# czbiohub-sf/yogo

Measured on AMD Instinct MI355X. Metric: training images/sec (772x1032 gray), higher is better.
Workload: dtype bf16; 1 GPU; BASELINE configs[2]: full train step (fwd+loss+bwd+clamp+AdamW), base_model, 772x1032x1 uint8, 7 classes; per_gpu_batch=128, global_batch=128, parallelism=dp1

## Files before the change

### include/yogo_hip.h

```cpp
#ifndef YOGO_HIP_H
#define YOGO_HIP_H

#include <stddef.h>

#ifdef __cplusplus
extern "C" {
#endif

typedef void* yogo_stream_t;

const char* yogo_hip_last_error(void);
int yogo_hip_abi_version(void);
int yogo_hip_launch_log(int enable);
int yogo_hip_launch_log_read(char* buf, size_t cap, size_t* needed);


int yogo_conv_packed_bytes(int Cin, int Cout, int ksize, int stride, int mode, size_t* bytes);
int yogo_conv_pack_f32(const float* w_oihw, float* packed, int Cin, int Cout, int ksize, int stride, int mode,
                       yogo_stream_t stream);
int yogo_conv2d_fwd_stats_shape(int B, int Cin, int Cout, int IH, int IW, int ksize, int stride, int* rows, int* mpad);
int yogo_conv2d_fwd_f32(const float* in, const float* packed, const float* bias, float* out, float* out_pre,
                        const float* chan_scale, float* stats_part, int B, int Cin, int Cout, int IH, int IW, int ksize,
                        int stride, int act, yogo_stream_t stream);
int yogo_conv2d_dgrad_f32(const float* dy, const float* packed_dgrad, float* dx, const float* act_ref, int ref_act,
// ... 54 lines not shown
                                     yogo_stream_t stream);
int yogo_head1x1_decode_fwd_bf16(const void* x, const void* packed, const float* bias, float* out, const float* cxs, const float* cys,
                                 int B, int Cin, int P, int Sy, int Sx, float anchor_w, float anchor_h, float width_multiplier,
                                 float height_multiplier, int inference, yogo_stream_t stream);

int yogo_match_workspace_bytes(int B, int Sy, int Sx, int cap, size_t* bytes);
int yogo_match_preds_labels_batched(const float* rows, const int* counts, const float* labels, int* meta, int* pair_label,
                                    int* pair_pred, int* un_label, int* un_pred, float* lab_out, void* workspace, int B, int P, int Sy,
                                    int Sx, int cap, yogo_stream_t stream);
int yogo_match_gather(const float* rows, const float* lab_out, const int* meta, const int* pair_label, const int* pair_pred,
                      const int* un_label, const int* un_pred, float* preds, float* labels, float* missed, float* extra, int B, int P,
                      int cap, long long K, long long Km, long long Ke, yogo_stream_t stream);
int yogo_metrics_state_layout(int C, int T, int nbins, long long* offsets);
int yogo_metrics_accumulate(const float* rows, const float* lab_out, const int* meta, const int* pair_label, const int* pair_pred,
                            const int* un_label, const int* un_pred, const double* roc_thresholds, int T, const double* cal_edges,
                            int nbins, long long* acc, double* bin_conf, double* partial, float* map_rows, long long map_cap, int B,
                            int P, int cap, yogo_stream_t stream);

int yogo_bf16_channel_blocks(int C);
int yogo_conv_bf16_packed_bytes(int Cin, int Cout, int ksize, int mode, size_t* bytes);
int yogo_conv_bf16_pack(const float* w_oihw, const float* scale, void* packed, int Cin, int Cout, int ksize, int mode,
                        yogo_stream_t stream);
int yogo_conv2d_fwd_bf16_stats_shape(int B, int Cin, int Cout, int IH, int IW, int ksize, int stride, int* rows, int* mpad);
int yogo_conv2d_fwd_bf16(const void* in, const void* packed, const float* bias, void* out, float* out_f32,
                         const float* chan_scale, float* stats_part, int B, int Cin, int Cout, int IH, int IW, int ksize,
                         int stride, int act, yogo_stream_t stream);
int yogo_conv2d_fwd_bf16_pre(const void* in, const void* packed, const float* bias, void* out, void* out_pre,
                             const float* chan_scale, int B, int Cin, int Cout, int IH, int IW, int ksize, int stride, int act,
                             yogo_stream_t stream);
int yogo_conv_bf16_pack_blocks(int Cin, int Cout, int ksize, int mode, int* blocks);
int yogo_conv_bf16_pack_multi(const void* table, int n, int total_blocks, yogo_stream_t stream);
int yogo_bf16_signs_bytes(int B, int C, int H, int W, size_t* bytes);
int yogo_conv2d_fwd_bf16_signs(const void* in, const void* packed, const float* bias, void* out, void* signs,
                               const float* chan_scale, int B, int Cin, int Cout, int IH, int IW, int ksize, int stride, int act,
                               yogo_stream_t stream);
int yogo_conv2d_dgrad_bf16_signs(const void* dy, const void* packed_dgrad, void* dx, const void* signs,
                                 const float* chan_scale, int B, int Cin, int Cout, int IH, int IW, int ksize, int stride,
                                 yogo_stream_t stream);
int yogo_conv2d_dgrad_bf16(const void* dy, const void* packed_dgrad, void* dx, const void* act_ref, int ref_act,
                           const float* chan_scale, int B, int Cin, int Cout, int IH, int IW, int ksize, int stride,
                           yogo_stream_t stream);
int yogo_conv2d_wgrad_bf16in(const void* x, const void* g, float* dw, float* db, void* workspace, int B, int Cin, int Cout,
                             int IH, int IW, int ksize, int stride, float clip, yogo_stream_t stream);
int yogo_conv2d_wgrad_bf16_workspace_bytes(int B, int Cin, int Cout, int IH, int IW, int ksize, int stride, size_t* bytes);
int yogo_conv2d_wgrad_bf16(const void* x, const void* g, float* dw, float* db, void* workspace, int B, int Cin, int Cout,
                           int IH, int IW, int ksize, int stride, float clip, yogo_stream_t stream);
// ... 102 lines not shown
```

### yogo_amd/csrc/conv_bf16.hip

```cpp
#include "common.h"
#include "conv_bf16_ws.h"
#include "conv_bf16_ws16.h"
#include "conv_bf16_ws3.h"
#include <type_traits>
#include <utility>
#include <cstdlib>
#include <vector>

typedef float f32x16 __attribute__((ext_vector_type(16)));
typedef __bf16 bf16x8 __attribute__((ext_vector_type(8)));
typedef __bf16 bf16x4 __attribute__((ext_vector_type(4)));
typedef unsigned int u32x4 __attribute__((ext_vector_type(4)));
typedef unsigned int u32x2 __attribute__((ext_vector_type(2)));
typedef int i32x16 __attribute__((ext_vector_type(16)));

#define BF_MAX_TAPS 9
#define BF_LDS_BUDGET (80 * 1024)
#define BF_LDS_MAX (160 * 1024)

struct ConvBf16Params {
  const u32x4* in;
  const u32x4* wp;
  const float* bias;
  u32x2* out;
// ... 1211 lines not shown
      if constexpr (REF != 1) {
        if (!general) {
          bf_launch_one<MW, NW, NWV, S2D, PF, F32, REF, true, true>(grid, lds_bytes, stream, p, plan_txt);
          return;
        }
      }
#else
      (void)general;
#endif
      bf_launch_one<MW, NW, NWV, S2D, PF, F32, REF, true>(grid, lds_bytes, stream, p, plan_txt);
      return;
    }
  }
  if constexpr (NWV == 4 && S2D && !F32 && REF != 1) {
    const bool general = p.stats_part != nullptr || p.act == ACT_SILU || p.out_pre != nullptr || (REF == 2 && p.ref_act != ACT_LEAKY);
    if (!general) {
      bf_launch_one<MW, NW, NWV, S2D, PF, F32, REF, false, true>(grid, lds_bytes, stream, p, plan_txt);
      return;
    }
  }
  bf_launch_one<MW, NW, NWV, S2D, PF, F32, REF, false>(grid, lds_bytes, stream, p, plan_txt);
}

int launch_conv_bf16(const void* in, const void* packed, const float* bias, void* out, float* out_f32, void* out_pre, const void* act_ref,
                     int ref_act, void* signs, bool signs_read, const float* chan_scale, float* stats_part, int B, int K, int M, int IH, int IW, int OH,
                     int OW, int ks, int a, int s2d, int act, hipStream_t stream, int* stats_rows, int* stats_mpad) {
  const int T = ks * ks, pad = ks == 3 ? 1 : 0;
  if (in != nullptr && g_bf_ws && !s2d && a == 1 && ks == 3 && out_f32 == nullptr && out_pre == nullptr && act_ref == nullptr && !signs_read &&
      stats_part == nullptr && (act == ACT_NONE || act == ACT_LEAKY) && !(signs != nullptr && act != ACT_LEAKY) &&
      conv_bf16_ws_eligible(K, M, IH, IW, B)) {
    ConvWsParams q{};
    q.in = in; q.wp = packed; q.bias = bias; q.out = out; q.signs = reinterpret_cast<unsigned char*>(signs); q.chan_scale = chan_scale;
    q.B = B; q.Kb = bf_kb_of(K); q.IH = IH; q.IW = IW; q.act = act;
#ifdef YOGO_DIAG
    q.dbg = g_diag_dbg;
    q.stamps = (g_diag_stamps != nullptr && g_diag_stamps_bytes >= 512 * 128) ? g_diag_stamps : nullptr;
    if (q.stamps) (void)hipMemsetAsync(g_diag_stamps, 0, 512 * 128, stream);
#endif
    if (conv_bf16_ws_plan(&q)) {
      if ((g_bf_ws16 == 2 || (g_bf_ws16 == 1 && bias == nullptr)) && act == ACT_NONE && signs == nullptr && chan_scale == nullptr &&
          conv_bf16_ws16_eligible(K, M, IH, IW, B))
        return launch_conv_bf16_ws16(q, stream);
      return launch_conv_bf16_ws(q, stream);
    }
  }
  if (in != nullptr && g_bf_ws && !s2d && a == 2 && ks == 3 && out_f32 == nullptr && out_pre == nullptr && act_ref == nullptr && !signs_read &&
      stats_part == nullptr && (act == ACT_NONE || act == ACT_LEAKY) && !(signs != nullptr && act != ACT_LEAKY) && conv_bf16_ws3_eligible(K, M, IH, IW, B)) {
    ConvWs3Params q{};
    q.in = in; q.wp = packed; q.bias = bias; q.out = out; q.signs = reinterpret_cast<unsigned char*>(signs); q.chan_scale = chan_scale;
    q.B = B; q.Kb = bf_kb_of(K); q.IH = IH; q.IW = IW; q.OH = OH; q.OW = OW; q.act = act;
#ifdef YOGO_DIAG
    q.dbg = g_diag_dbg;
    q.stamps = (g_diag_stamps != nullptr && g_diag_stamps_bytes >= 512 * 128) ? g_diag_stamps : nullptr;
    if (q.stamps) (void)hipMemsetAsync(g_diag_stamps, 0, 512 * 128, stream);
#endif
    if (conv_bf16_ws3_plan(&q)) return launch_conv_bf16_ws3(q, stream);
  }
  if (in != nullptr && g_bf_head && ks == 1 && a == 1 && !s2d && out_pre == nullptr && act_ref == nullptr && stats_part == nullptr && act == ACT_NONE &&
      out_f32 != nullptr && out == nullptr && signs == nullptr && chan_scale == nullptr && conv_bf16_head_fwd_eligible(K, M, OH * OW, B))
    return launch_conv_bf16_head_fwd(in, packed, bias, out_f32, B, K, M, OH * OW, stream);
  if (in != nullptr && g_bf_staged && !s2d && ks == 3 && out_f32 == nullptr && out_pre == nullptr && act_ref == nullptr && !signs_read && stats_part == nullptr &&
      (act == ACT_NONE || act == ACT_LEAKY) && !(signs != nullptr && act != ACT_LEAKY) && conv_bf16_staged_eligible(K, M, a, IH, IW, OH, OW, B))
    return launch_conv_bf16_staged(in, packed, bias, out, signs, chan_scale, B, K, M, IH, IW, OH, OW, a, act, stream);
  if (in != nullptr && g_bf_direct && s2d && ks == 3 && out_f32 == nullptr && out_pre == nullptr && act_ref == nullptr && bias == nullptr &&
      stats_part == nullptr && act == ACT_NONE && (!signs_read || (signs != nullptr && ref_act == ACT_LEAKY)) && (signs_read || signs == nullptr) &&
      conv_bf16_s2d_direct_eligible(K, M, OH, OW, B))
    return launch_conv_bf16_s2d_direct(in, packed, out, signs_read ? signs : nullptr, chan_scale, B, K, M, IH, IW, OH, OW, stream);
  const int MW = bf_pick_mw(M);
  const bool small_n = s2d || a == 2;
  const bool wide64 = MW == 2 && !small_n && K >= 64 && OH * OW >= 4096;
  const int NW = MW == 1 ? (small_n ? 2 : 4) : (small_n ? 1 : (wide64 ? 4 : 2));
  const int NWV = (MW == 4 || wide64) ? 8 : 4;
  const int PF = NWV == 8 ? 10 : 16;
  const int Kb = bf_kb_of(K), Mpad = bf_mpad_of(M);
  const int OHt = s2d ? (OH + 1) / 2 : OH, OWt = s2d ? (OW + 1) / 2 : OW;
  BfTiling tl;
  bool planned = false;
  if (NWV == 4) {
    const int ladder[3] = {40 * 1024, 53 * 1024, BF_LDS_BUDGET};
// ... 101 lines not shown
    else if (MW == 2) BFLAUNCH(2, 1, 4, false, 16);
    else BFLAUNCH(1, 2, 4, false, 16);
  } else {
    if (MW == 4) BFLAUNCH(4, 2, 8, false, 10);
    else if (MW == 2 && wide64) BFLAUNCH(2, 4, 8, false, 10);
    else if (MW == 2) BFLAUNCH(2, 2, 4, false, 16);
    else BFLAUNCH(1, 4, 4, false, 16);
  }
#undef BFLAUNCH
#undef BFLAUNCH_
#undef BFLAUNCH__
  YOGO_CHECK_LAUNCH("conv_bf16");
  return YOGO_OK;
}

int check_bf16_conv(int B, int Cin, int Cout, int IH, int IW, int ks, int stride) {
  YOGO_CHECK_ARG((ks == 3 || ks == 1) && (stride == 1 || stride == 2) && !(ks == 1 && stride != 1) && B >= 0 && Cin > 0 &&
                     Cout > 0 && IH > 0 && IW > 0, "conv_bf16: unsupported shape");
  return YOGO_OK;
}

}

extern "C" int yogo_conv2d_fwd_bf16_stats_shape(int B, int Cin, int Cout, int IH, int IW, int ks, int stride, int* rows, int* mpad) {
  if (int e = check_bf16_conv(B, Cin, Cout, IH, IW, ks, stride)) return e;
  const int pad = ks == 3 ? 1 : 0;
  return launch_conv_bf16(nullptr, nullptr, nullptr, nullptr, nullptr, nullptr, nullptr, 0, nullptr, false, nullptr, nullptr, B, Cin, Cout, IH, IW,
                          (IH + 2 * pad - ks) / stride + 1, (IW + 2 * pad - ks) / stride + 1, ks, stride, 0, 0, nullptr, rows, mpad);
}

extern "C" int yogo_conv2d_fwd_bf16(const void* in, const void* packed, const float* bias, void* out, float* out_f32,
                                    const float* chan_scale, float* stats_part, int B, int Cin, int Cout, int IH, int IW,
                                    int ks, int stride, int act, hipStream_t stream) {
  YOGO_CHECK_ARG(in && packed && (out || out_f32), "conv2d_fwd_bf16: null pointer");
  if (int e = check_bf16_conv(B, Cin, Cout, IH, IW, ks, stride)) return e;
  const int pad = ks == 3 ? 1 : 0;
  return launch_conv_bf16(in, packed, bias, out, out_f32, nullptr, nullptr, 0, nullptr, false, chan_scale, stats_part, B, Cin, Cout, IH, IW,
                          (IH + 2 * pad - ks) / stride + 1, (IW + 2 * pad - ks) / stride + 1, ks, stride, 0, act, stream,
                          nullptr, nullptr);
}

extern "C" int yogo_conv2d_fwd_bf16_pre(const void* in, const void* packed, const float* bias, void* out, void* out_pre,
                                        const float* chan_scale, int B, int Cin, int Cout, int IH, int IW, int ks, int stride,
                                        int act, hipStream_t stream) {
  YOGO_CHECK_ARG(in && packed && out && out_pre, "conv2d_fwd_bf16_pre: null pointer");
  if (int e = check_bf16_conv(B, Cin, Cout, IH, IW, ks, stride)) return e;
// ... 65 lines not shown
```

### yogo_amd/csrc/conv_bf16_ws3.h

```cpp
#pragma once
#include "common.h"

#define W3_PT 128
#define W3_ROWS 9
#define W3_PL 48
#define W3_LW (2 * W3_PL)
#define W3_KBU (W3_ROWS * W3_LW)
#define W3_IB (2 * W3_KBU * 16)
#define W3_NI 7
#define W3_WB (9 * 4096)
#define W3_I0 (2 * W3_WB)
#define W3_EB (W3_I0 + 3 * W3_IB)
#define W3_ES (W3_EB + 512)
#define W3_LDS_BYTES (W3_ES + 1024)

struct ConvWs3Params {
  const void* in;
  const void* wp;
  const float* bias;
  void* out;
  unsigned char* signs;
  const float* chan_scale;
  int B, Kb, IH, IW, OH, OW;
  int ncb, TW, tiles_per_band, gx, ntiles;
  int PT;
  unsigned m_gx, m_tpb, m_bw, m_bwl;
  int nchunk, act;
#ifdef YOGO_DIAG
  int dbg;
  unsigned long long* stamps;
#endif
};

bool conv_bf16_ws3_eligible(int K, int M, int IH, int IW, int B);
bool conv_bf16_ws3_plan(ConvWs3Params* p);
int launch_conv_bf16_ws3(const ConvWs3Params& p, hipStream_t stream);
```

### yogo_amd/csrc/conv_bf16_ws3.hip

```cpp
#include "conv_bf16_ws3.h"
#include <mutex>
#include <type_traits>
#include <utility>

typedef unsigned int u32x4 __attribute__((ext_vector_type(4)));
typedef int i32x4 __attribute__((ext_vector_type(4)));
typedef __bf16 bf16x8 __attribute__((ext_vector_type(8)));

namespace {

__device__ __forceinline__ int w3_udivm(int n, unsigned m) { return (int)__umulhi((unsigned)n, m); }
__device__ __forceinline__ int w3_udivm1(int n, int d, unsigned m) { return d == 1 ? n : (int)__umulhi((unsigned)n, m); }
__device__ __forceinline__ int w3_lane() {
  int l;
  asm volatile("v_mbcnt_lo_u32_b32 %0, -1, 0\n\tv_mbcnt_hi_u32_b32 %0, -1, %0" : "=v"(l));
  return l;
}
__device__ __forceinline__ i32x4 w3_rsrc(const void* ptr, unsigned bytes) {
  const unsigned long long a = reinterpret_cast<unsigned long long>(ptr);
  return i32x4{(int)(unsigned)a, (int)((unsigned)(a >> 32) & 0xFFFFu), (int)bytes, 0x00020000};
}
__device__ __forceinline__ unsigned w3_u(unsigned x) { return (unsigned)__builtin_amdgcn_readfirstlane((int)x); }
__device__ __forceinline__ i32x4 w3_u4(i32x4 r) {
  return i32x4{__builtin_amdgcn_readfirstlane(r.x), __builtin_amdgcn_readfirstlane(r.y), __builtin_amdgcn_readfirstlane(r.z), __builtin_amdgcn_readfirstlane(r.w)};
}
__device__ __forceinline__ void w3_dma9(i32x4 rs, unsigned lds, int voff, unsigned soff, unsigned step) {
  unsigned so;
  rs = w3_u4(rs); lds = w3_u(lds); soff = w3_u(soff); step = w3_u(step);
#define W3_P9 "s_add_u32 m0, m0, 4096\n\ts_add_u32 %0, %0, %5\n\tbuffer_load_dwordx4 %1, %2, %0 offen lds\n\t"
  asm volatile("s_mov_b32 m0, %3\n\ts_mov_b32 %0, %4\n\ts_nop 4\n\tbuffer_load_dwordx4 %1, %2, %0 offen lds\n\t" W3_P9 W3_P9 W3_P9 W3_P9 W3_P9 W3_P9 W3_P9 W3_P9
// ... 78 lines not shown
               : "memory", W3_ACC_CLOBBER);
}
__device__ __forceinline__ void w3_k_end(const u32x4& a0, const u32x4& a1, const u32x4& b0, const u32x4& b1) {
  asm volatile(W3_MF(0, a0, b0) W3_MF(1, a0, b1) W3_MF(2, a1, b0) W3_MF(3, a1, b1) "s_nop 15\n\ts_nop 15" : : W3_OPS_IN : "memory", W3_ACC_CLOBBER);
}
template <int BIMM0, int BIMM1>
__device__ __forceinline__ void w3_k_first(u32x4& an0, u32x4& an1, u32x4& bn0, u32x4& bn1, u32x4& am0, u32x4& am1, u32x4& bm0, u32x4& bm1, unsigned pa, unsigned pb0,
                                           unsigned pb1) {
  asm volatile(W3_RD(an0, pa, z0) W3_RD(an1, pa, z512) W3_RD(bn0, pb0, bo0) W3_RD(bn1, pb1, bo0) W3_RD(am0, pa, z4096) W3_RD(am1, pa, z4608) W3_RD(bm0, pb0, bo1)
               W3_RD(bm1, pb1, bo1) "s_waitcnt lgkmcnt(4)"
               : [an0] "=&v"(an0), [an1] "=&v"(an1), [bn0] "=&v"(bn0), [bn1] "=&v"(bn1), [am0] "=&v"(am0), [am1] "=&v"(am1), [bm0] "=&v"(bm0), [bm1] "=&v"(bm1)
               : [pa] "v"(pa), [pb0] "v"(pb0), [pb1] "v"(pb1), [z0] "n"(0), [z512] "n"(512), [z4096] "n"(4096), [z4608] "n"(4608), [bo0] "n"(BIMM0), [bo1] "n"(BIMM1)
               : "memory");
}
template <int R>
__device__ __forceinline__ void w3_acc_read8(float (&r)[8]) {
  asm volatile(
      "v_accvgpr_read_b32 %0, a[%8]\n\tv_accvgpr_read_b32 %1, a[%8+1]\n\tv_accvgpr_read_b32 %2, a[%8+2]\n\tv_accvgpr_read_b32 %3, a[%8+3]\n\t"
      "v_accvgpr_read_b32 %4, a[%8+4]\n\tv_accvgpr_read_b32 %5, a[%8+5]\n\tv_accvgpr_read_b32 %6, a[%8+6]\n\tv_accvgpr_read_b32 %7, a[%8+7]"
      : "=v"(r[0]), "=v"(r[1]), "=v"(r[2]), "=v"(r[3]), "=v"(r[4]), "=v"(r[5]), "=v"(r[6]), "=v"(r[7])
      : "n"(R)
      : W3_ACC_CLOBBER);
}
__device__ constexpr int w3_bimm(int t) { return ((t / 3) * W3_LW + ((t % 3) == 1 ? 0 : W3_PL + ((t % 3) == 2 ? 1 : 0))) * 16; }

template <class F, int... I>
__device__ __forceinline__ void w3_static_for(F&& f, std::integer_sequence<int, I...>) {
  (f(std::integral_constant<int, I>{}), ...);
}

#ifdef YOGO_DIAG
#define W3_DBG(BIT) (p.dbg & (BIT))
#define W3_STAMP() __builtin_amdgcn_s_memtime()
#else
#define W3_DBG(BIT) 0
#define W3_STAMP() 0ull
#endif

}

template <int MODE>
__global__ __launch_bounds__(512) __attribute__((amdgpu_waves_per_eu(2, 2))) void conv_bf16_ws3_kernel(const ConvWs3Params p) {
  extern __shared__ __attribute__((aligned(16))) u32x4 smem4[];
  constexpr unsigned OOB = 0x80000000u;
  float* const ldsf = reinterpret_cast<float*>(smem4);
  const int tid = threadIdx.x;
  const int wave = __builtin_amdgcn_readfirstlane(tid >> 6);
// ... 10 lines not shown
  struct TileS { int b, j0, bw, p0, p1, lastband; };
  auto find_tile = [&](unsigned& k, TileS& t) __attribute__((always_inline)) -> bool {
    for (;; ++k) {
      const unsigned lin = slot + k * G;
      if (lin >= NV) return false;
      const unsigned xcd = lin & 7;
      const int widx = (int)((xcd < xr ? xcd * (xq + 1) : xr * (xq + 1) + (xcd - xr) * xq) + (lin >> 3));
      const int b = w3_udivm1(widx, p.gx, p.m_gx);
      const int bx = widx - b * p.gx;
      const int cb = w3_udivm1(bx, p.tiles_per_band, p.m_tpb);
      const int tb = bx - cb * p.tiles_per_band;
      const int j0 = cb * p.TW;
      const int bw = min(p.TW, OW - j0);
      const int NPb = OH * bw;
      const int p0 = tb * p.PT;
      if (p0 >= NPb) continue;
      t.b = b; t.j0 = j0; t.bw = bw; t.p0 = p0; t.p1 = min(p0 + p.PT, NPb); t.lastband = cb == p.ncb - 1;
      return true;
    }
  };

  unsigned k_ord = 0;
  TileS T{};
  if (!find_tile(k_ord, T)) return;
  if (tid < 128) {
    ldsf[W3_EB / 4 + tid] = p.bias != nullptr ? p.bias[tid] : 0.f;
    if (p.chan_scale == nullptr) {
      ldsf[W3_ES / 4 + tid] = 1.f;
      ldsf[W3_ES / 4 + 128 + tid] = 1.f;
    }
  }
  __syncthreads();

  if (team == 1) {
    const int lane = w3_lane();
    const int ttid = tw * 64 + lane;
    const int rowb = IW * 16, kcb = IH * IW * 16;
    const unsigned ibytes = (unsigned)p.Kb * kcb, wbytes = 9u * p.Kb * 2048u;
    const unsigned so_i = 2u * kcb;
    const unsigned wstep = (unsigned)p.Kb * 2048u;
    const i32x4 rs_w = w3_rsrc(p.wp, wbytes);
    const int lane16 = W3_DBG(4) ? (int)OOB : lane * 16;
    const bool has_scale = p.chan_scale != nullptr;
    const i32x4 rs_sc = w3_rsrc(p.chan_scale, has_scale ? (unsigned)p.B * 512u : 0u);
    auto issue_scale = [&](int b, int par) __attribute__((always_inline)) {
      if (has_scale && tw < 2) w3_dma_dword(rs_sc, (unsigned)(W3_ES + par * 512 + tw * 256), lane * 4, (unsigned)((b * 128 + tw * 64) * 4));
    };
// ... 87 lines not shown

  const int lane = w3_lane(), l31 = lane & 31, half = lane >> 5;
  const unsigned a_b0 = (unsigned)(half * 128 + mh * 64 + l31) * 16u;
  const unsigned obytes = 16u * plane16;
  unsigned pbr[2];
  int vo[2];
  auto decode_pix = [&](const TileS& t) __attribute__((always_inline)) {
    const unsigned m_bw = t.lastband ? p.m_bwl : p.m_bw;
    const int bw = t.bw;
    const int i_lo = w3_udivm1(t.p0, bw, m_bw);
#pragma unroll
    for (int n = 0; n < 2; ++n) {
      const int pp = t.p0 + (nh * 2 + n) * 32 + l31;
      const bool pv = pp < t.p1;
      const int pc = pv ? pp : (t.p1 - 1);
      const int i = w3_udivm1(pc, bw, m_bw), j = pc - i * bw;
      pbr[n] = (unsigned)(2 * (i - i_lo) * W3_LW + j + half * W3_KBU) * 16u;
      vo[n] = (pv && !W3_DBG(1)) ? (i * OW + t.j0 + j) * 16 + half * plane16 : (int)OOB;
    }
  };
  decode_pix(T);
  u32x4 A[3][2], B[3][2];
  int tpar = 0;
  auto epilogue = [&](i32x4 rs_o) __attribute__((always_inline)) {
    if constexpr ((W3_ABL & 8) != 0) return;
    [[maybe_unused]] unsigned sg[2] = {0u, 0u};
    w3_static_for([&](auto q_tag) __attribute__((always_inline)) {
      constexpr int Q = decltype(q_tag)::value, MB = Q >> 1, GP = Q & 1;
      const int cl = mh * 64 + MB * 32 + 16 * GP + 4 * half;
      const float* eb = ldsf + W3_EB / 4 + cl;
      const float4 bA = *reinterpret_cast<const float4*>(eb), bB = *reinterpret_cast<const float4*>(eb + 8);
      const float ba[8] = {bA.x, bA.y, bA.z, bA.w, bB.x, bB.y, bB.z, bB.w};
      float sa[8] = {1.f, 1.f, 1.f, 1.f, 1.f, 1.f, 1.f, 1.f}, bs[8];
      if constexpr (SCALED) {
        const float* es = ldsf + W3_ES / 4 + tpar * 128 + cl;
        const float4 sA = *reinterpret_cast<const float4*>(es), sB = *reinterpret_cast<const float4*>(es + 8);
        sa[0] = sA.x; sa[1] = sA.y; sa[2] = sA.z; sa[3] = sA.w; sa[4] = sB.x; sa[5] = sB.y; sa[6] = sB.z; sa[7] = sB.w;
      }
#pragma unroll
      for (int i = 0; i < 8; ++i) bs[i] = SCALED ? ba[i] * sa[i] : ba[i];
      const unsigned so = (unsigned)(mh * 8 + MB * 4 + GP * 2) * (unsigned)plane16;
      w3_static_for([&](auto n_tag) __attribute__((always_inline)) {
        constexpr int n = decltype(n_tag)::value;
        float v[8], r[8];
        w3_acc_read8<16 * (2 * MB + n) + 8 * GP>(r);
#pragma unroll
        for (int i = 0; i < 8; ++i) v[i] = SCALED ? fmaf(r[i], sa[i], bs[i]) : r[i] + bs[i];
        if constexpr (leaky) {
          float sv[8];
#pragma unroll
          for (int i = 0; i < 8; ++i) sv[i] = v[i] * LEAKY_SLOPE;
#pragma unroll
          for (int i = 0; i < 8; ++i) asm("v_max_f32 %0, %0, %1" : "+v"(v[i]) : "v"(sv[i]));
        }
        if constexpr (write_signs) {
          unsigned mA = 0;
#define W3_SGN(I) "v_cmp_lt_f32_e32 vcc, 0, %" #I "\n\tv_addc_co_u32_e32 %0, vcc, %0, %0, vcc\n\t"
          asm(W3_SGN(8) W3_SGN(7) W3_SGN(6) W3_SGN(5) W3_SGN(4) W3_SGN(3) W3_SGN(2) "v_cmp_lt_f32_e32 vcc, 0, %1\n\tv_addc_co_u32_e32 %0, vcc, %0, %0, vcc"
              : "+v"(mA)
              : "v"(v[0]), "v"(v[1]), "v"(v[2]), "v"(v[3]), "v"(v[4]), "v"(v[5]), "v"(v[6]), "v"(v[7])
              : "vcc");
#undef W3_SGN
          sg[n] |= mA << (8 * Q);
        }
        if (W3_DBG(2)) {
#pragma unroll
          for (int i = 0; i < 8; ++i) v[i] = r[i];
        }
        bf16x8 o;
#pragma unroll
        for (int i = 0; i < 8; ++i) o[i] = (__bf16)v[i];
        const u32x4 w = __builtin_bit_cast(u32x4, o);
        const auto r0 = __builtin_amdgcn_permlane32_swap(w.x, w.z, false, false);
        const auto r1 = __builtin_amdgcn_permlane32_swap(w.y, w.w, false, false);
        const u32x4 st = {r0[0], r1[0], r0[1], r1[1]};
        w3_store16(st, vo[n], rs_o, so);
      }, std::make_integer_sequence<int, 2>{});
    }, std::make_integer_sequence<int, 4>{});
    if constexpr (write_signs) {
      const i32x4 rs_s = w3_rsrc(p.signs + (size_t)T.b * plane * 16, (unsigned)plane * 16u);
#pragma unroll
      for (int n = 0; n < 2; ++n) {
        const int vs = vo[n] < 0 ? (int)OOB : (vo[n] >> 1) + mh * 4;
        asm volatile("s_nop 4\n\tbuffer_store_dword %0, %1, %2, 0 offen\n\ts_nop 1" ::"v"(sg[n]), "v"(vs), "s"(w3_u4(rs_s)) : "memory");
      }
    }
  };
  auto period = [&](auto first_tag, auto last_tag, unsigned pa, unsigned pan, unsigned ib, unsigned ibn) __attribute__((always_inline)) {
    constexpr bool FIRST = decltype(first_tag)::value, LASTP = decltype(last_tag)::value;
    const unsigned pb0 = pbr[0] + ib, pb1 = pbr[1] + ib;
    w3_static_for([&](auto s_tag) __attribute__((always_inline)) {
      constexpr int S = decltype(s_tag)::value;
      u32x4(&Ac)[2] = A[S % 3];
      u32x4(&Bc)[2] = B[S % 3];
      if constexpr (S < 7) {
        constexpr int S2 = S + 2;
        w3_k_rd<FIRST && S == 0, S2 * 4096, w3_bimm(S2)>(Ac[0], Ac[1], Bc[0], Bc[1], A[S2 % 3][0], A[S2 % 3][1], B[S2 % 3][0], B[S2 % 3][1], pa, pb0, pb1);
      } else if constexpr (S == 7) {
        w3_k_bar(Ac[0], Ac[1], Bc[0], Bc[1], A[2][0], A[2][1], B[2][0], B[2][1]);
      } else if constexpr (!LASTP) {
// ... 15 lines not shown
    const i32x4 rs_o = w3_rsrc(reinterpret_cast<unsigned char*>(p.out) + (size_t)T.b * obytes, obytes);
    [[maybe_unused]] const unsigned long long s0 = W3_STAMP();
    w3_k_first<w3_bimm(0), w3_bimm(1)>(A[0][0], A[0][1], B[0][0], B[0][1], A[1][0], A[1][1], B[1][0], B[1][1], (unsigned)(wpar * W3_WB) + a_b0, pbr[0] + ibo, pbr[1] + ibo);
    for (int c = 0; c < nck; ++c) {
      const unsigned pa = (unsigned)(wpar * W3_WB) + a_b0, pan = (unsigned)((wpar ^ 1) * W3_WB) + a_b0;
      const unsigned ibn = ibo == W3_I0 + 2 * W3_IB ? (unsigned)W3_I0 : ibo + W3_IB;
      if (c == 0) period(TT{}, FT{}, pa, pan, ibo, ibn);
      else if (c == nck - 1) period(FT{}, TT{}, pa, pan, ibo, ibn);
      else period(FT{}, FT{}, pa, pan, ibo, ibn);
      wpar ^= 1;
      ibo = ibn;
    }
    [[maybe_unused]] const unsigned long long s1 = W3_STAMP();
    epilogue(rs_o);
    [[maybe_unused]] const unsigned long long s2 = W3_STAMP();
    t_k += s1 - s0; t_e += s2 - s1;
    unsigned kn = k_ord + 1;
    const bool has_next = find_tile(kn, T);
    k_ord = kn;
    if (!has_next) break;
    decode_pix(T);
    tpar ^= 1;
  }
#ifdef YOGO_DIAG
  if (p.stamps && tw == 0 && lane == 0) {
    unsigned long long* d = p.stamps + (size_t)blockIdx.x * 16;
    d[0] = t_start; d[1] = __builtin_amdgcn_s_memtime(); d[2] = t_k; d[3] = t_e; d[6] = k_ord;
  }
#endif
}

bool conv_bf16_ws3_eligible(int K, int M, int IH, int IW, int B) {
  const int Kb = round_up(K, 16) / 8;
  if (M != 128 || Kb < 8 || (Kb % 4) != 0) return false;
  if (IH < 3 || IW < 3 || B <= 0) return false;
  const long long OH = (IH - 1) / 2 + 1, OW = (IW - 1) / 2 + 1;
  if ((long long)Kb * IH * IW * 16 >= (1ll << 31) || 16ll * OH * OW * 16 >= (1ll << 31)) return false;
  return true;
}

bool conv_bf16_ws3_plan(ConvWs3Params* p) {
  const int OH = p->OH, OW = p->OW;
  long long best = -1;
  int best_ncb = 0, best_pt = 0;
  for (int ncb = 1; ncb <= 64 && ncb <= OW; ++ncb) {
    const int TW = cdiv(OW, ncb);
// ... 1 lines not shown
    const int bw_min = OW - (ncb - 1) * TW;
    const int pt = OH <= 4 ? W3_PT : min(W3_PT, 3 * bw_min + 1);
    const long long tiles = (long long)(ncb - 1) * cdiv(OH * TW, pt) + cdiv(OH * bw_min, pt);
    if (best < 0 || tiles < best) { best = tiles; best_ncb = ncb; best_pt = pt; }
  }
  if (best < 0) return false;
  p->ncb = best_ncb;
  p->TW = cdiv(OW, best_ncb);
  p->PT = best_pt;
  p->tiles_per_band = cdiv(OH * p->TW, p->PT);
  p->gx = p->ncb * p->tiles_per_band;
  p->ntiles = p->B * p->gx;
  auto magic = [](int d) -> unsigned { return d <= 1 ? 0xFFFFFFFFu : (unsigned)(((1ull << 32) + (unsigned)d - 1ull) / (unsigned)d); };
  const int bw_last = OW - (p->ncb - 1) * p->TW;
  p->m_gx = magic(p->gx); p->m_tpb = magic(p->tiles_per_band);
  p->m_bw = magic(p->TW); p->m_bwl = magic(bw_last);
  p->nchunk = p->Kb / 2;
  if (!magic_div_exact((long long)p->ntiles - 1, p->gx) || !magic_div_exact(p->gx, p->tiles_per_band) || !magic_div_exact((long long)OH * p->TW, p->TW) ||
      !magic_div_exact((long long)OH * bw_last, bw_last))
    return false;
  return true;
}

int launch_conv_bf16_ws3(const ConvWs3Params& p, hipStream_t stream) {
  static std::mutex mu;
  static int n_cu_of[64] = {0};
  int dev = 0;
  if (hipGetDevice(&dev) != hipSuccess || dev < 0 || dev >= 64) {
    yogo_set_error("conv_bf16_ws3: hipGetDevice failed");
    return YOGO_ERR_HIP;
  }
  int n_cu;
  {
    std::lock_guard<std::mutex> lk(mu);
    if (n_cu_of[dev] == 0) {
      hipError_t e = hipSuccess;
#define W3_ATTR(M) if (e == hipSuccess) e = hipFuncSetAttribute(reinterpret_cast<const void*>(&conv_bf16_ws3_kernel<M>), hipFuncAttributeMaxDynamicSharedMemorySize, W3_LDS_BYTES);
      W3_ATTR(0) W3_ATTR(1) W3_ATTR(2) W3_ATTR(3) W3_ATTR(5) W3_ATTR(7)
#undef W3_ATTR
      if (e != hipSuccess) {
        yogo_set_error("conv_bf16_ws3: hipFuncSetAttribute(MaxDynamicSharedMemorySize = %d) failed: %s", W3_LDS_BYTES, hipGetErrorString(e));
        return YOGO_ERR_HIP;
      }
      hipDeviceProp_t prop;
      n_cu_of[dev] = (hipGetDeviceProperties(&prop, dev) == hipSuccess && prop.multiProcessorCount > 0) ? prop.multiProcessorCount : 256;
    }
    n_cu = n_cu_of[dev];
  }
  if (p.ntiles <= 0) return YOGO_OK;
  int grid = min(p.ntiles, n_cu);
  if (grid >= 8) grid &= ~7;
  const int mode = (p.act == ACT_LEAKY ? 1 : 0) | (p.chan_scale != nullptr ? 2 : 0) | (p.signs != nullptr ? 4 : 0);
#define W3_LAUNCH(M) case M: hipLaunchKernelGGL(conv_bf16_ws3_kernel<M>, dim3(grid), dim3(512), W3_LDS_BYTES, stream, p); break;
  switch (mode) { W3_LAUNCH(0) W3_LAUNCH(1) W3_LAUNCH(2) W3_LAUNCH(3) W3_LAUNCH(5) W3_LAUNCH(7) }
#undef W3_LAUNCH
  if (yogo_launch_log_enabled())
    yogo_launch_log("conv_bf16_ws3_kernel<%d> | Kb=%d in=%dx%d out=%dx%d ncb=%d TW=%d PT=%d tiles_per_band=%d nchunk=%d ntiles=%d grid=%d lds=%d act=%d scale=%d signs=%d", mode, p.Kb,
                    p.IH, p.IW, p.OH, p.OW, p.ncb, p.TW, p.PT, p.tiles_per_band, p.nchunk, p.ntiles, grid, W3_LDS_BYTES, p.act, p.chan_scale != nullptr, p.signs != nullptr);
  YOGO_CHECK_LAUNCH("conv_bf16_ws3");
  return YOGO_OK;
}
```

### yogo_amd/engine.py

```python
from __future__ import annotations

import threading
import weakref
from dataclasses import dataclass, field
from typing import Dict, List, Optional, Tuple

import torch
from torch import nn

from yogo_amd import _hip

ACT_NONE, ACT_LEAKY, ACT_SILU = 0, 1, 2


@dataclass
class Layer:
    conv: nn.Conv2d
    bn: Optional[nn.BatchNorm2d] = None
    act: int = ACT_NONE
    drop: Optional[nn.Dropout2d] = None

    @property
    def cin(self) -> int:
        return self.conv.in_channels
# ... 287 lines not shown
                _hip.call("yogo_conv2d_dgrad_f32", g, pk, dx, act_ref, ref_act, Sp.mask, B, L.cin, L.cout, IH, IW, L.k, L.s, st)
                self._tock()
                g = dx
        bb = self.backbone_ref()
        return [grads.get(id(p)) for p in bb.parameters()]



def _blocks(c: int) -> int:
    return ((c + 15) // 16) * 2


_WGRAD_BF16_MFMA = True
_WGRAD_SIDE_STREAM = False
_FUSE_LAYER0_BWD = True
_LEAKY_SIGNS = True
_L0_MFMA = True
_L0_GRAM = True
_WGRAD_DEFER_REDUCE = True
_L0_NO_Z = True
_PACK_MULTI = True
_L01_FUSE_BWD = True
_HEAD_BN_FUSE = True
_BN_STATS_PASS = True
_SIDE_STREAMS: Dict[int, "torch.cuda.Stream"] = {}


def _side_stream(dev: torch.device) -> "torch.cuda.Stream":
    key = dev.index if dev.index is not None else torch.cuda.current_device()
    if key not in _SIDE_STREAMS:
        _SIDE_STREAMS[key] = torch.cuda.Stream(device=dev)
    return _SIDE_STREAMS[key]


def _packed_bf16(eng: Engine, i: int, mode: int) -> torch.Tensor:
    L = eng.layers[i]
    w = L.conv.weight
    key = (i, 10 + mode)
    hit = eng._pack.get(key)
    if hit is not None and hit[0] == w._version and hit[1] == w.data_ptr():
        return hit[2]
    nbytes = _hip.query_size("yogo_conv_bf16_packed_bytes", L.cin, L.cout, L.k, mode)
    buf = torch.empty(nbytes, dtype=torch.uint8, device=w.device)
    _hip.call("yogo_conv_bf16_pack", _f32(w.detach()), None, buf, L.cin, L.cout, L.k, mode, _hip.stream_ptr())
    eng._pack[key] = (w._version, w.data_ptr(), buf)
    return buf

# ... 120 lines not shown
                    eng.generation += 1
            else:
                invstd = torch.empty(L.cout, dtype=torch.float32, device=dev)
                _hip.call("yogo_bn_invstd", bn.running_var, float(bn.eps), invstd, L.cout, st)
                mean = bn.running_mean
            no_z = (_L0_NO_Z and _FUSE_LAYER0_BWD and S.gram is not None and L.conv.bias is None
                    and _hip.lib().yogo_conv_first_bn_wgrad_xs_supported(0, L.cin, L.cout, H, W, L.s, L.act))
            if no_z:
                out8 = None
                S.signs0 = torch.empty(B, OH * OW * 2, dtype=torch.uint8, device=dev)
                _hip.call("yogo_conv_first_mfma_signs", cur, w32, bias, None, y, S.signs0, mean, invstd, gamma, beta, B, L.cout, H, W, L.act, st)
            else:
                out8 = torch.empty_like(y)
                _hip.call("yogo_conv_first_mfma", cur, w32, bias, out8, y, mean, invstd, gamma, beta, None, B, L.cout, H, W, L.act, st)
            S.mean, S.invstd, S.bn_train, S.z, S.y = mean, invstd, bn_train, out8, y
            S.w_used = w32.to(torch.bfloat16).to(torch.float32)
            cur = y
            saved.append(S)
            H, W = OH, OW
            continue
        fused_act = ACT_NONE if has_bn else L.act
        stats = None
        rows = mpad = 0
        stats_pass = bn_train and i > 0 and _BN_STATS_PASS
        if bn_train and not stats_pass:
            if i == 0:
                rows, mpad = _hip.query_ints("yogo_conv_first_stats_rows", 1, B, H, W, L.s)[0], L.cout
            else:
                rows, mpad = _hip.query_ints("yogo_conv2d_fwd_bf16_stats_shape", 2, B, L.cin, L.cout, H, W, L.k, L.s)
            stats = torch.empty(rows * mpad * 2, dtype=torch.float32, device=dev)
        out8 = None if last else torch.empty(B, _blocks(L.cout), OH, OW, 8, dtype=torch.bfloat16, device=dev)
        out32 = torch.empty(B, L.cout, OH, OW, dtype=torch.float32, device=dev) if last else None
        if last and (has_bn or mask is not None):
            raise RuntimeError("yogo_amd: BatchNorm / Dropout on the last layer is not supported by the bf16 path")
        if i == 0:
            _hip.call("yogo_conv_first_fwd_train_bf16", cur, 0 if cur.dtype == torch.uint8 else 1, _f32(L.conv.weight.detach()), bias,
                      out8, mask, stats, B, L.cin, L.cout, H, W, L.s, fused_act, st)
        else:
            pk = _packed_bf16(eng, i, 0)
            nbytes = B * (_blocks(L.cin) * 8 * H * W * 2 + (L.cout * OH * OW * 4 if last else _blocks(L.cout) * 8 * OH * OW * 2))
            eng._tick("fwd", i, 2.0 * B * L.cout * L.cin * L.k * L.k * OH * OW, mw=34 if (L.cout > 64 and L.s == 1) else (35 if (L.cout > 64 and L.cin > 64 and L.k == 3) else 30), nbytes=nbytes)
            if silu_pre:
                S.pre = torch.empty_like(out8)
                _hip.call("yogo_conv2d_fwd_bf16_pre", cur, pk, bias, out8, S.pre, mask, B, L.cin, L.cout, H, W, L.k, L.s, fused_act, st)
            elif _LEAKY_SIGNS and L.act == ACT_LEAKY and not has_bn and not last:
                S.signs = torch.empty(_hip.query_size("yogo_bf16_signs_bytes", B, L.cout, OH, OW), dtype=torch.uint8, device=dev)
                _hip.call("yogo_conv2d_fwd_bf16_signs", cur, pk, bias, out8, S.signs, mask, B, L.cin, L.cout, H, W, L.k, L.s, fused_act, st)
            else:
                _hip.call("yogo_conv2d_fwd_bf16", cur, pk, bias, out8, out32, mask, stats, B, L.cin, L.cout, H, W, L.k, L.s, fused_act, st)
            eng._tock()
        if has_bn:
            bn = L.bn
# ... 479 lines not shown
```

Before: 11280 images/s.

## Fuse BatchNorm partial statistics into the stride-2 ws3 conv epilogue

```diff
diff --git a/include/yogo_hip.h b/include/yogo_hip.h
--- a/include/yogo_hip.h
+++ b/include/yogo_hip.h
@@ -100,6 +100,8 @@
 int yogo_conv_bf16_pack(const float* w_oihw, const float* scale, void* packed, int Cin, int Cout, int ksize, int mode,
                         yogo_stream_t stream);
 int yogo_conv2d_fwd_bf16_stats_shape(int B, int Cin, int Cout, int IH, int IW, int ksize, int stride, int* rows, int* mpad);
+int yogo_conv2d_fwd_bf16_stats_plan(int B, int Cin, int Cout, int IH, int IW, int ksize, int stride, int act, int has_scale, int* producer,
+                                    int* rows, int* mpad);
 int yogo_conv2d_fwd_bf16(const void* in, const void* packed, const float* bias, void* out, float* out_f32,
                          const float* chan_scale, float* stats_part, int B, int Cin, int Cout, int IH, int IW, int ksize,
                          int stride, int act, yogo_stream_t stream);
diff --git a/yogo_amd/csrc/conv_bf16.hip b/yogo_amd/csrc/conv_bf16.hip
--- a/yogo_amd/csrc/conv_bf16.hip
+++ b/yogo_amd/csrc/conv_bf16.hip
@@ -1257,6 +1257,14 @@
   bf_launch_one<MW, NW, NWV, S2D, PF, F32, REF, false>(grid, lds_bytes, stream, p, plan_txt);
 }
 
+bool bf_ws3_takes(bool stats, int act, bool scale, bool signs, int s2d, int a, int ks, int B, int K, int M, int IH, int IW, int OH, int OW, ConvWs3Params* q) {
+  if (!g_bf_ws || s2d || a != 2 || ks != 3 || !(act == ACT_NONE || act == ACT_LEAKY) || (signs && act != ACT_LEAKY)) return false;
+  if (stats && (act != ACT_NONE || scale || signs)) return false;
+  if (!conv_bf16_ws3_eligible(K, M, IH, IW, B)) return false;
+  q->B = B; q->Kb = bf_kb_of(K); q->IH = IH; q->IW = IW; q->OH = OH; q->OW = OW; q->act = act;
+  return conv_bf16_ws3_plan(q);
+}
+
 int launch_conv_bf16(const void* in, const void* packed, const float* bias, void* out, float* out_f32, void* out_pre, const void* act_ref,
                      int ref_act, void* signs, bool signs_read, const float* chan_scale, float* stats_part, int B, int K, int M, int IH, int IW, int OH,
                      int OW, int ks, int a, int s2d, int act, hipStream_t stream, int* stats_rows, int* stats_mpad) {
@@ -1279,17 +1287,19 @@
       return launch_conv_bf16_ws(q, stream);
     }
   }
-  if (in != nullptr && g_bf_ws && !s2d && a == 2 && ks == 3 && out_f32 == nullptr && out_pre == nullptr && act_ref == nullptr && !signs_read &&
-      stats_part == nullptr && (act == ACT_NONE || act == ACT_LEAKY) && !(signs != nullptr && act != ACT_LEAKY) && conv_bf16_ws3_eligible(K, M, IH, IW, B)) {
+  {
     ConvWs3Params q{};
-    q.in = in; q.wp = packed; q.bias = bias; q.out = out; q.signs = reinterpret_cast<unsigned char*>(signs); q.chan_scale = chan_scale;
-    q.B = B; q.Kb = bf_kb_of(K); q.IH = IH; q.IW = IW; q.OH = OH; q.OW = OW; q.act = act;
+    if (in != nullptr && out_f32 == nullptr && out_pre == nullptr && act_ref == nullptr && !signs_read &&
+        bf_ws3_takes(stats_part != nullptr, act, chan_scale != nullptr, signs != nullptr, s2d, a, ks, B, K, M, IH, IW, OH, OW, &q)) {
+      q.in = in; q.wp = packed; q.bias = bias; q.out = out; q.signs = reinterpret_cast<unsigned char*>(signs); q.chan_scale = chan_scale;
+      q.stats_part = stats_part;
 #ifdef YOGO_DIAG
-    q.dbg = g_diag_dbg;
-    q.stamps = (g_diag_stamps != nullptr && g_diag_stamps_bytes >= 512 * 128) ? g_diag_stamps : nullptr;
-    if (q.stamps) (void)hipMemsetAsync(g_diag_stamps, 0, 512 * 128, stream);
-#endif
-    if (conv_bf16_ws3_plan(&q)) return launch_conv_bf16_ws3(q, stream);
+      q.dbg = g_diag_dbg;
+      q.stamps = (g_diag_stamps != nullptr && g_diag_stamps_bytes >= 512 * 128) ? g_diag_stamps : nullptr;
+      if (q.stamps) (void)hipMemsetAsync(g_diag_stamps, 0, 512 * 128, stream);
+#endif
+      return launch_conv_bf16_ws3(q, stream);
+    }
   }
   if (in != nullptr && g_bf_head && ks == 1 && a == 1 && !s2d && out_pre == nullptr && act_ref == nullptr && stats_part == nullptr && act == ACT_NONE &&
       out_f32 != nullptr && out == nullptr && signs == nullptr && chan_scale == nullptr && conv_bf16_head_fwd_eligible(K, M, OH * OW, B))
@@ -1437,6 +1447,23 @@
 
 }
 
+extern "C" int yogo_conv2d_fwd_bf16_stats_plan(int B, int Cin, int Cout, int IH, int IW, int ks, int stride, int act, int has_scale, int* producer,
+                                               int* rows, int* mpad) {
+  YOGO_CHECK_ARG(producer && rows && mpad, "conv2d_fwd_bf16_stats_plan: null pointer");
+  if (int e = check_bf16_conv(B, Cin, Cout, IH, IW, ks, stride)) return e;
+  const int pad = ks == 3 ? 1 : 0;
+  const int OH = (IH + 2 * pad - ks) / stride + 1, OW = (IW + 2 * pad - ks) / stride + 1;
+  ConvWs3Params q{};
+  if (bf_ws3_takes(true, act, has_scale != 0, false, 0, stride, ks, B, Cin, Cout, IH, IW, OH, OW, &q)) {
+    *producer = 1;
+    *mpad = 128;
+    return conv_bf16_ws3_stats_rows(q, rows);
+  }
+  *producer = 0;
+  return launch_conv_bf16(nullptr, nullptr, nullptr, nullptr, nullptr, nullptr, nullptr, 0, nullptr, false, nullptr, nullptr, B, Cin, Cout, IH, IW, OH, OW, ks,
+                          stride, 0, 0, nullptr, rows, mpad);
+}
+
 extern "C" int yogo_conv2d_fwd_bf16_stats_shape(int B, int Cin, int Cout, int IH, int IW, int ks, int stride, int* rows, int* mpad) {
   if (int e = check_bf16_conv(B, Cin, Cout, IH, IW, ks, stride)) return e;
   const int pad = ks == 3 ? 1 : 0;
diff --git a/yogo_amd/csrc/conv_bf16_ws3.h b/yogo_amd/csrc/conv_bf16_ws3.h
--- a/yogo_amd/csrc/conv_bf16_ws3.h
+++ b/yogo_amd/csrc/conv_bf16_ws3.h
@@ -21,6 +21,7 @@
   void* out;
   unsigned char* signs;
   const float* chan_scale;
+  float* stats_part;
   int B, Kb, IH, IW, OH, OW;
   int ncb, TW, tiles_per_band, gx, ntiles;
   int PT;
@@ -35,3 +36,4 @@
 bool conv_bf16_ws3_eligible(int K, int M, int IH, int IW, int B);
 bool conv_bf16_ws3_plan(ConvWs3Params* p);
 int launch_conv_bf16_ws3(const ConvWs3Params& p, hipStream_t stream);
+int conv_bf16_ws3_stats_rows(const ConvWs3Params& p, int* rows);
diff --git a/yogo_amd/csrc/conv_bf16_ws3.hip b/yogo_amd/csrc/conv_bf16_ws3.hip
--- a/yogo_amd/csrc/conv_bf16_ws3.hip
+++ b/yogo_amd/csrc/conv_bf16_ws3.hip
@@ -6,6 +6,7 @@
 typedef unsigned int u32x4 __attribute__((ext_vector_type(4)));
 typedef int i32x4 __attribute__((ext_vector_type(4)));
 typedef __bf16 bf16x8 __attribute__((ext_vector_type(8)));
+typedef float f32x2 __attribute__((ext_vector_type(2)));
 
 namespace {
 
@@ -130,7 +131,44 @@
       : "n"(R)
       : W3_ACC_CLOBBER);
 }
+#define W3_STAT_CLOBBER "a64","a65","a66","a67","a68","a69","a70","a71","a72","a73","a74","a75","a76","a77","a78","a79","a80","a81","a82","a83","a84","a85","a86","a87","a88","a89","a90","a91","a92","a93","a94","a95","a96","a97","a98","a99","a100","a101","a102","a103","a104","a105","a106","a107","a108","a109","a110","a111","a112","a113","a114","a115","a116","a117","a118","a119","a120","a121","a122","a123","a124","a125","a126","a127"
+__device__ __forceinline__ void w3_stat_zero() {
+#define W3_Z8(R) "v_accvgpr_write_b32 a[" #R "], 0\n\tv_accvgpr_write_b32 a[" #R "+1], 0\n\tv_accvgpr_write_b32 a[" #R "+2], 0\n\tv_accvgpr_write_b32 a[" #R "+3], 0\n\t" \
+                 "v_accvgpr_write_b32 a[" #R "+4], 0\n\tv_accvgpr_write_b32 a[" #R "+5], 0\n\tv_accvgpr_write_b32 a[" #R "+6], 0\n\tv_accvgpr_write_b32 a[" #R "+7], 0\n\t"
+  asm volatile(W3_Z8(64) W3_Z8(72) W3_Z8(80) W3_Z8(88) W3_Z8(96) W3_Z8(104) W3_Z8(112) W3_Z8(120) "s_nop 0" ::: W3_STAT_CLOBBER);
+#undef W3_Z8
+}
+template <int R>
+__device__ __forceinline__ void w3_stat_read8(float (&r)[8]) {
+  asm volatile(
+      "v_accvgpr_read_b32 %0, a[%8]\n\tv_accvgpr_read_b32 %1, a[%8+1]\n\tv_accvgpr_read_b32 %2, a[%8+2]\n\tv_accvgpr_read_b32 %3, a[%8+3]\n\t"
+      "v_accvgpr_read_b32 %4, a[%8+4]\n\tv_accvgpr_read_b32 %5, a[%8+5]\n\tv_accvgpr_read_b32 %6, a[%8+6]\n\tv_accvgpr_read_b32 %7, a[%8+7]\n\t"
+      "s_nop 1"
+      : "=v"(r[0]), "=v"(r[1]), "=v"(r[2]), "=v"(r[3]), "=v"(r[4]), "=v"(r[5]), "=v"(r[6]), "=v"(r[7])
+      : "n"(R)
+      : W3_STAT_CLOBBER);
+}
+template <int R>
+__device__ __forceinline__ void w3_stat_write8(const float (&r)[8]) {
+  asm volatile(
+      "v_accvgpr_write_b32 a[%8], %0\n\tv_accvgpr_write_b32 a[%8+1], %1\n\tv_accvgpr_write_b32 a[%8+2], %2\n\tv_accvgpr_write_b32 a[%8+3], %3\n\t"
+      "v_accvgpr_write_b32 a[%8+4], %4\n\tv_accvgpr_write_b32 a[%8+5], %5\n\tv_accvgpr_write_b32 a[%8+6], %6\n\tv_accvgpr_write_b32 a[%8+7], %7"
+      :
+      : "v"(r[0]), "v"(r[1]), "v"(r[2]), "v"(r[3]), "v"(r[4]), "v"(r[5]), "v"(r[6]), "v"(r[7]), "n"(R)
+      : W3_STAT_CLOBBER);
+}
 __device__ constexpr int w3_bimm(int t) { return ((t / 3) * W3_LW + ((t % 3) == 1 ? 0 : W3_PL + ((t % 3) == 2 ? 1 : 0))) * 16; }
+
+__device__ __forceinline__ float w3_half_sum(float v) {
+#define W3_DPP_ADD(CTRL, ROWMASK) v += __builtin_bit_cast(float, __builtin_amdgcn_update_dpp(0, __builtin_bit_cast(int, v), CTRL, ROWMASK, 0xf, false));
+  W3_DPP_ADD(0xB1, 0xf)
+  W3_DPP_ADD(0x4E, 0xf)
+  W3_DPP_ADD(0x141, 0xf)
+  W3_DPP_ADD(0x140, 0xf)
+  W3_DPP_ADD(0x142, 0xa)
+#undef W3_DPP_ADD
+  return v;
+}
 
 template <class F, int... I>
 __device__ __forceinline__ void w3_static_for(F&& f, std::integer_sequence<int, I...>) {
@@ -187,7 +225,10 @@
 
   unsigned k_ord = 0;
   TileS T{};
-  if (!find_tile(k_ord, T)) return;
+  if (!find_tile(k_ord, T)) {
+    if (p.stats_part != nullptr) p.stats_part[(size_t)blockIdx.x * 512 + tid] = 0.f;
+    return;
+  }
   if (tid < 128) {
     ldsf[W3_EB / 4 + tid] = p.bias != nullptr ? p.bias[tid] : 0.f;
     if (p.chan_scale == nullptr) {
@@ -321,6 +362,10 @@
   decode_pix(T);
   u32x4 A[3][2], B[3][2];
   int tpar = 0;
+  const bool do_stats = MODE == 0 && p.stats_part != nullptr;
+  if constexpr (MODE == 0) {
+    if (do_stats) w3_stat_zero();
+  }
   auto epilogue = [&](i32x4 rs_o) __attribute__((always_inline)) {
     if constexpr ((W3_ABL & 8) != 0) return;
     [[maybe_unused]] unsigned sg[2] = {0u, 0u};
@@ -339,6 +384,7 @@
 #pragma unroll
       for (int i = 0; i < 8; ++i) bs[i] = SCALED ? ba[i] * sa[i] : ba[i];
       const unsigned so = (unsigned)(mh * 8 + MB * 4 + GP * 2) * (unsigned)plane16;
+      [[maybe_unused]] u32x4 st_w[2];
       w3_static_for([&](auto n_tag) __attribute__((always_inline)) {
         constexpr int n = decltype(n_tag)::value;
         float v[8], r[8];
@@ -370,11 +416,32 @@
 #pragma unroll
         for (int i = 0; i < 8; ++i) o[i] = (__bf16)v[i];
         const u32x4 w = __builtin_bit_cast(u32x4, o);
+        if constexpr (MODE == 0) {
+          if (do_stats) st_w[n] = vo[n] >= 0 ? w : u32x4{0u, 0u, 0u, 0u};
+        }
         const auto r0 = __builtin_amdgcn_permlane32_swap(w.x, w.z, false, false);
         const auto r1 = __builtin_amdgcn_permlane32_swap(w.y, w.w, false, false);
         const u32x4 st = {r0[0], r1[0], r0[1], r1[1]};
         w3_store16(st, vo[n], rs_o, so);
       }, std::make_integer_sequence<int, 2>{});
+      if constexpr (MODE == 0) {
+        if (do_stats) {
+          float ss[8], sq[8];
+          w3_stat_read8<64 + 8 * Q>(ss);
+          w3_stat_read8<96 + 8 * Q>(sq);
+#pragma unroll
+          for (int i = 0; i < 4; ++i) {
+            const f32x2 x0 = {__uint_as_float(st_w[0][i] << 16), __uint_as_float(st_w[0][i] & 0xFFFF0000u)};
+            const f32x2 x1 = {__uint_as_float(st_w[1][i] << 16), __uint_as_float(st_w[1][i] & 0xFFFF0000u)};
+            const f32x2 a = f32x2{ss[2 * i], ss[2 * i + 1]} + (x0 + x1);
+            const f32x2 b = __builtin_elementwise_fma(x1, x1, __builtin_elementwise_fma(x0, x0, f32x2{sq[2 * i], sq[2 * i + 1]}));
+            ss[2 * i] = a[0]; ss[2 * i + 1] = a[1];
+            sq[2 * i] = b[0]; sq[2 * i + 1] = b[1];
+          }
+          w3_stat_write8<64 + 8 * Q>(ss);
+          w3_stat_write8<96 + 8 * Q>(sq);
+        }
+      }
     }, std::make_integer_sequence<int, 4>{});
     if constexpr (write_signs) {
       const i32x4 rs_s = w3_rsrc(p.signs + (size_t)T.b * plane * 16, (unsigned)plane * 16u);
@@ -436,6 +503,23 @@
     decode_pix(T);
     tpar ^= 1;
   }
+  if constexpr (MODE == 0) {
+    if (do_stats) {
+      float* const row = p.stats_part + ((size_t)blockIdx.x * 2 + nh) * 256;
+      w3_static_for([&](auto q_tag) __attribute__((always_inline)) {
+        constexpr int Q = decltype(q_tag)::value, MB = Q >> 1, GP = Q & 1;
+        const int cl = mh * 64 + MB * 32 + 16 * GP + 4 * half;
+        float ss[8], sq[8];
+        w3_stat_read8<64 + 8 * Q>(ss);
+        w3_stat_read8<96 + 8 * Q>(sq);
+#pragma unroll
+        for (int i = 0; i < 8; ++i) {
+          const float s = w3_half_sum(ss[i]), q = w3_half_sum(sq[i]);
+          if (l31 == 31) *reinterpret_cast<float2*>(row + (cl + (i < 4 ? i : i + 4)) * 2) = make_float2(s, q);
+        }
+      }, std::make_integer_sequence<int, 4>{});
+    }
+  }
 #ifdef YOGO_DIAG
   if (p.stamps && tw == 0 && lane == 0) {
     unsigned long long* d = p.stamps + (size_t)blockIdx.x * 16;
@@ -483,7 +567,7 @@
   return true;
 }
 
-int launch_conv_bf16_ws3(const ConvWs3Params& p, hipStream_t stream) {
+static int w3_grid(const ConvWs3Params& p, int* grid_out) {
   static std::mutex mu;
   static int n_cu_of[64] = {0};
   int dev = 0;
@@ -508,16 +592,34 @@
     }
     n_cu = n_cu_of[dev];
   }
+  int grid = min(max(p.ntiles, 0), n_cu);
+  if (grid >= 8) grid &= ~7;
+  *grid_out = grid;
+  return YOGO_OK;
+}
+
+int conv_bf16_ws3_stats_rows(const ConvWs3Params& p, int* rows) {
+  int grid = 0;
+  if (int e = w3_grid(p, &grid)) return e;
+  *rows = 2 * grid;
+  return YOGO_OK;
+}
+
+int launch_conv_bf16_ws3(const ConvWs3Params& p, hipStream_t stream) {
+  int grid = 0;
+  if (int e = w3_grid(p, &grid)) return e;
   if (p.ntiles <= 0) return YOGO_OK;
-  int grid = min(p.ntiles, n_cu);
-  if (grid >= 8) grid &= ~7;
   const int mode = (p.act == ACT_LEAKY ? 1 : 0) | (p.chan_scale != nullptr ? 2 : 0) | (p.signs != nullptr ? 4 : 0);
+  if (p.stats_part != nullptr && mode != 0) {
+    yogo_set_error("conv_bf16_ws3: partial sums go with the plain epilogue (no activation, channel scale or sign map)");
+    return YOGO_ERR_ARG;
+  }
 #define W3_LAUNCH(M) case M: hipLaunchKernelGGL(conv_bf16_ws3_kernel<M>, dim3(grid), dim3(512), W3_LDS_BYTES, stream, p); break;
   switch (mode) { W3_LAUNCH(0) W3_LAUNCH(1) W3_LAUNCH(2) W3_LAUNCH(3) W3_LAUNCH(5) W3_LAUNCH(7) }
 #undef W3_LAUNCH
   if (yogo_launch_log_enabled())
-    yogo_launch_log("conv_bf16_ws3_kernel<%d> | Kb=%d in=%dx%d out=%dx%d ncb=%d TW=%d PT=%d tiles_per_band=%d nchunk=%d ntiles=%d grid=%d lds=%d act=%d scale=%d signs=%d", mode, p.Kb,
-                    p.IH, p.IW, p.OH, p.OW, p.ncb, p.TW, p.PT, p.tiles_per_band, p.nchunk, p.ntiles, grid, W3_LDS_BYTES, p.act, p.chan_scale != nullptr, p.signs != nullptr);
+    yogo_launch_log("conv_bf16_ws3_kernel<%d> | Kb=%d in=%dx%d out=%dx%d ncb=%d TW=%d PT=%d tiles_per_band=%d nchunk=%d ntiles=%d grid=%d lds=%d act=%d scale=%d signs=%d stats=%d", mode, p.Kb,
+                    p.IH, p.IW, p.OH, p.OW, p.ncb, p.TW, p.PT, p.tiles_per_band, p.nchunk, p.ntiles, grid, W3_LDS_BYTES, p.act, p.chan_scale != nullptr, p.signs != nullptr, p.stats_part != nullptr);
   YOGO_CHECK_LAUNCH("conv_bf16_ws3");
   return YOGO_OK;
 }
diff --git a/yogo_amd/engine.py b/yogo_amd/engine.py
--- a/yogo_amd/engine.py
+++ b/yogo_amd/engine.py
@@ -333,7 +333,7 @@
 _PACK_MULTI = True
 _L01_FUSE_BWD = True
 _HEAD_BN_FUSE = True
-_BN_STATS_PASS = True
+_BN_STATS_PASS = False
 _SIDE_STREAMS: Dict[int, "torch.cuda.Stream"] = {}
 
 
@@ -500,12 +500,13 @@
         fused_act = ACT_NONE if has_bn else L.act
         stats = None
         rows = mpad = 0
-        stats_pass = bn_train and i > 0 and _BN_STATS_PASS
+        stats_pass = bn_train and i > 0
+        if stats_pass and not _BN_STATS_PASS and not last and mask is None and not silu_pre:
+            producer, rows, mpad = _hip.query_ints("yogo_conv2d_fwd_bf16_stats_plan", 3, B, L.cin, L.cout, H, W, L.k, L.s, fused_act, 0)
+            stats_pass = not producer
         if bn_train and not stats_pass:
             if i == 0:
                 rows, mpad = _hip.query_ints("yogo_conv_first_stats_rows", 1, B, H, W, L.s)[0], L.cout
-            else:
-                rows, mpad = _hip.query_ints("yogo_conv2d_fwd_bf16_stats_shape", 2, B, L.cin, L.cout, H, W, L.k, L.s)
             stats = torch.empty(rows * mpad * 2, dtype=torch.float32, device=dev)
         out8 = None if last else torch.empty(B, _blocks(L.cout), OH, OW, 8, dtype=torch.bfloat16, device=dev)
         out32 = torch.empty(B, L.cout, OH, OW, dtype=torch.float32, device=dev) if last else None
```

Result: no change. 11320 images/s, median of 6 (+0.3%).
